# tuanggolt/hyperdrive

Hardware: AMD Instinct MI355X
Metric: verified consensus msgs/sec (secp256k1) at 1/2/4/8 MI355X; % INT32 VALU peak (higher is better)
Workload: dtype u32 (256-bit modular integer arithmetic)

## Files before the change

hyperdrive_amd/csrc/hd_fastverify.hip:

```cpp
#include <hip/hip_runtime.h>

#include <algorithm>
#include <cstdio>
#include <cstdlib>
#include <cstring>
#include <string>
#include <map>
#include <mutex>
#include <unordered_map>
#include <vector>

#include "../../include/hd_verify.h"
#include "hd_fixedbase.h"
#include "hd_dedup.h"
#include "hd_scmont.h"
#include "hd_internal.h"
#include "hd_verify_msg.h"

using namespace hd;

struct FbWork {
    const gp* gtab = nullptr;
    uint32_t nslots = 0;
    uint32_t max_slots = 0;
    gp** tabs = nullptr;
    std::vector<gp*> chunks;
    ge* base = nullptr;
    ge* pub = nullptr;
    uint32_t* state = nullptr;
    int32_t* adm_slot = nullptr;
    bool map_ok = true;
    size_t cap_adm_slot = 0;
    uint32_t* list = nullptr;
    uint32_t* counts = nullptr;
    uint32_t* zr = nullptr;
    struct Scratch {
        uint32_t* rows = nullptr;
        size_t cap_rows = 0;
        uint32_t* dtab = nullptr;
        size_t cap_dtab = 0;
        uint32_t* slow = nullptr;
        size_t cap_slow = 0;
        uint32_t* count = nullptr;
        uint32_t* slow2 = nullptr;
        size_t cap_slow2 = 0;
        hipEvent_t done = nullptr;
        hipStream_t stream = nullptr;
        bool used = false;
    };
    static constexpr int NSCRATCH = 3;
    Scratch sc[NSCRATCH];
    int next = 0;
    int last_set = -1;
    uint32_t* nr_host = nullptr;
    uint32_t* nr_dev = nullptr;
    uint32_t* est_host = nullptr;
    uint32_t* est_dev = nullptr;
    unsigned long long* dstats = nullptr;
    hipEvent_t done = nullptr;
    hipStream_t last = nullptr;
    bool any = false;
    bool steady = false;
    bool prof = false;
    std::vector<hipEvent_t> ev_call, ev_sums;
    size_t n_call = 0, n_sums = 0;
    std::unordered_map<std::string, uint32_t> slot_of;
    std::vector<uint32_t> free_slots;
    uint32_t used = 1;
    int wp = HD_FB_W;
    int last_k = 8;
    double budget = 0;
    size_t bytes = 0;
    uint32_t* fdict = nullptr;
    uint32_t* fnext = nullptr;
    uint32_t fbase = 0, fcap = 0, fres = 0;
    uint32_t* fpend_host = nullptr;
    uint32_t* fpend_dev = nullptr;
    uint32_t fseen = 0;
    uint32_t* fhit = nullptr;
    ge* fkey = nullptr;
    uint32_t fwait = 1, fcalls = 0;
    bool fforce = false;
    uint32_t evictions = 0;
    uint32_t evict_checks = 0;
    uint32_t evict_aborts = 0;
};

namespace {

#define FBCHK(expr, what)                                \
    do {                                                 \
        hipError_t e_ = (expr);                          \
        if (e_ != hipSuccess) return hd_ctx_fail(ctx, e_, what); \
    } while (0)

struct FastSrc {
    const DevBatch& b;
    uint32_t i;
    const uint8_t* dg;
    __device__ __forceinline__ uint32_t type() const { return b.type[i]; }
    __device__ __forceinline__ uint32_t value(int w) const { return load_be32(b.value32 + 32 * (size_t)i + 4 * w); }
    __device__ __forceinline__ uint32_t from(int w) const { return load_be32(b.from32 + 32 * (size_t)i + 4 * w); }
    __device__ __forceinline__ uint32_t sig_r(int w) const { return load_be32(b.sig65 + 65 * (size_t)i + 4 * w); }
    __device__ __forceinline__ uint32_t sig_s(int w) const { return load_be32(b.sig65 + 65 * (size_t)i + 32 + 4 * w); }
    __device__ __forceinline__ uint32_t sig_v() const { return b.sig65[65 * (size_t)i + 64]; }
    __device__ __forceinline__ void sig(uint32_t r_be[8], uint32_t s_be[8], uint32_t& v) const {
        load_sig65(r_be, s_be, v, b.sig65, i, b.n);
    }
    __device__ __forceinline__ void from_words(uint32_t w[8]) const { load_row32_be(w, b.from32, i); }
    __device__ __forceinline__ void value_words(uint32_t w[8]) const { load_row32_be(w, b.value32, i); }
};

#define HD_FAST_LIVE 0xFDu

template <int NW>
HD void soa_load(uint32_t (&w)[NW], const uint32_t* __restrict__ p, uint32_t n, uint32_t i) {
    HD_UNROLL for (int k = 0; k < NW; k++) w[k] = p[(size_t)k * n + i];
}
template <int NW>
HD void soa_store(uint32_t* __restrict__ p, uint32_t n, uint32_t i, const uint32_t (&w)[NW]) {
    HD_UNROLL for (int k = 0; k < NW; k++) p[(size_t)k * n + i] = w[k];
}

struct SplitRows {
    uint32_t* aux;
    int32_t* idx;
    uint32_t* ref;
    uint32_t* u1;
    uint32_t* u2;
    uint32_t* s;
    uint32_t* pre;
    uint32_t* xyz;
    uint32_t* cnt;
    int prio;
};

HD uint32_t dd_resolve(const SplitRows& rows, uint32_t i, uint32_t& c, bool& has_slot) {
    uint32_t rf = rows.ref[i];
    has_slot = (rf >> 30) != 3u;
    c = 0;
    if (!has_slot) return rf & 0xFFu;
    if (rf & HD_DD_REPEAT) rf = rows.ref[rf & HD_DD_INDEX];
    c = rf;
    return rows.aux[c] & 0xFFu;
}

HD void wave_prio(int p) {
    if (p == 1) __builtin_amdgcn_s_setprio(1);
    else if (p == 2) __builtin_amdgcn_s_setprio(2);
    else if (p >= 3) __builtin_amdgcn_s_setprio(3);
}

#define HD_REF_NEG 0x80000000u
#define HD_REF_ZERO 0x40000000u
#define HD_REF_IDX 0x3FFFFFFFu
template <int W>
HD uint32_t fb_ref(int d, int w) {
    const uint32_t ad = (uint32_t)(d < 0 ? -d : d);
    const uint32_t base = (uint32_t)w * FbL<W>::N;
    return d == 0 ? (base | HD_REF_ZERO) : ((base + ad - 1) | (d < 0 ? HD_REF_NEG : 0u));
}

__global__ __launch_bounds__(256) void k_fast_prep(DevBatch b, const uint8_t* __restrict__ digest_in,
                                                   const uint32_t* __restrict__ state,
                                                   const int32_t* __restrict__ adm_slot, AdmIndex ix,
                                                   uint32_t n_adm, SplitRows rows, const uint32_t* __restrict__ fdict,
                                                   uint32_t* __restrict__ fhit, uint32_t fbase,
                                                   uint32_t* __restrict__ dtab, uint32_t dmask) {
    wave_prio(rows.prio);
    const uint32_t i = blockIdx.x * blockDim.x + threadIdx.x;
    const uint32_t n = b.n;
    const bool present = i < n;
    FastSrc src{b, present ? i : 0u, digest_in};
    const uint32_t type = present ? src.type() : 0u;
    uint32_t code = HD_NEEDS_SLOW, slot = 0, rep = HD_DD_EMPTY;
    int32_t idx = -1;
    sc r, s, m;
    if (!present) {
    } else if (type < 1 || type > 3) {
        code = V_BAD_TYPE;
    } else {
        uint32_t from_be[8];
        src.from_words(from_be);
        idx = n_adm ? adm_index_find(ix, from_be) : -1;
        int32_t sl = idx >= 0 ? adm_slot[idx] : -1;
        if (idx < 0 && fdict) {
            sl = fdict_find(fdict, from_be);
            if (sl >= 0) idx = -2;
        }
        if (sl >= 0 && state[sl] == HD_FB_READY) {
            slot = (uint32_t)sl;
            if (idx == -2) atomicAdd(&fhit[sl - (int32_t)fbase], 1u);
            FastIn in;
            DdKey me;
            me.height = me.round = 0;
            if (digest_in) {
                load_row32_be(in.digest_be, digest_in, i);
                HD_UNROLL for (int k = 0; k < 8; k++) me.value[k] = in.digest_be[k];
            } else {
                src.value_words(me.value);
                me.height = b.height[i];
                me.round = b.round[i];
                if (type == T_PROPOSE)
                    sha256_propose(in.digest_be, me.height, me.round, b.valid_round ? b.valid_round[i] : -1, me.value);
                else
                    sha256_vote(in.digest_be, me.height, me.round, me.value);
            }
            src.sig(in.r_be, in.s_be, in.v);
            in.ready = true;
            fe x;
            uint8_t o;
            if (fast_prefix(o, r, s, m, x, in)) {
                code = HD_FAST_LIVE;
                if (dtab && type != T_PROPOSE) {
                    HD_UNROLL for (int k = 0; k < 8; k++) {
                        me.from[k] = from_be[k];
                        me.r[k] = in.r_be[k];
                        me.s[k] = in.s_be[k];
                    }
                    me.v = in.v;
                    const uint32_t h = dd_hash(me);
                    HD_NOUNROLL for (uint32_t p = 0; p < HD_DD_PROBES; p++) {
                        const uint32_t cur = atomicCAS(&dtab[(h + p) & dmask], HD_DD_EMPTY, i);
                        if (cur == HD_DD_EMPTY) break;
                        DdKey other;
                        dd_key_load(other, b.height, b.round, b.value32, digest_in, b.from32, b.sig65, cur, n);
                        if (dd_key_equal(me, other)) {
                            rep = cur;
                            break;
                        }
                    }
                }
            } else {
                code = o;
            }
        }
    }
    const bool live = code == HD_FAST_LIVE;
    const bool distinct = live && rep == HD_DD_EMPTY;
    __shared__ uint32_t s_cnt[4], s_base;
    const uint32_t lane = threadIdx.x & 63u, wv = threadIdx.x >> 6;
    const unsigned long long bd = __ballot(distinct), br = __ballot(live && !distinct);
    if (lane == 0) s_cnt[wv] = (uint32_t)__popcll(bd) | (uint32_t)__popcll(br) << 16;
    __syncthreads();
    if (threadIdx.x == 0) {
        const uint32_t t = s_cnt[0] + s_cnt[1] + s_cnt[2] + s_cnt[3];
        s_base = 0;
        if (t)
            s_base = (uint32_t)atomicAdd((unsigned long long*)(rows.cnt + 2),
                                         (unsigned long long)(t & 0xFFFFu) | (unsigned long long)(t >> 16) << 32);
    }
    __syncthreads();
    if (!present) return;
    if (distinct) {
        uint32_t c = s_base + (uint32_t)__popcll(bd & ((1ull << lane) - 1ull));
        for (uint32_t w = 0; w < wv; w++) c += s_cnt[w] & 0xFFFFu;
        rows.aux[c] = slot << 8 | HD_FAST_LIVE;
        soa_store(rows.u1, n, c, m.v);
        soa_store(rows.u2, n, c, r.v);
        soa_store(rows.s, n, c, s.v);
        rows.ref[i] = c;
    } else {
        rows.ref[i] = live ? (HD_DD_REPEAT | rep) : (HD_DD_FINAL | code);
    }
    rows.idx[i] = idx;
}

template <int K>
HD uint32_t split_lanes(uint32_t nc) {
    return ((nc + (uint32_t)K - 1) / (uint32_t)K + 63u) & ~63u;
}

template <int K>
__global__ __launch_bounds__(256) void k_fast_sinv(uint32_t n, SplitRows rows, uint32_t* __restrict__ est,
                                                   unsigned long long* __restrict__ stats) {
    wave_prio(rows.prio);
    const uint32_t t = blockIdx.x * blockDim.x + threadIdx.x;
    const uint32_t nc = rows.cnt[2], T = split_lanes<K>(nc);
    if (t == 0) {
        const uint32_t reps = rows.cnt[3];
        if (est) {
            est[1] = n;
            est[0] = nc;
        }
        if (nc + reps) atomicAdd(&stats[0], (unsigned long long)nc + reps);
        if (reps) atomicAdd(&stats[1], (unsigned long long)reps);
    }
    if (t >= T) return;
    sc sv[K];
    uint32_t live = 0;
    static_for<K>([&](auto jc) {
        constexpr int j = decltype(jc)::value;
        const uint32_t i = (uint32_t)j * T + t;
        const uint32_t ic = i < nc ? i : nc - 1;
        const uint32_t a = rows.aux[ic];
        soa_load(sv[j].v, rows.s, n, ic);
        live |= (i < nc && (a & 0xFFu) == HD_FAST_LIVE) ? 1u << j : 0u;
    });
    if (!live) return;
    sm pre[K], acc;
    HD_UNROLL for (int k = 0; k < 9; k++) acc.n[k] = 0;
    static_for<K>([&](auto jc) {
        constexpr int j = decltype(jc)::value;
        if ((live >> j) & 1u) {
            sm ss;
            sm_from_sc(ss, sv[j]);
            if (live & ((1u << j) - 1u)) sm_mul(acc, acc, ss);
            else acc = ss;
        }
        pre[j] = acc;
    });
    sm inv;
    {
        sc p, pinv;
        sm_to_sc(p, acc);
        sc_inv_divsteps(pinv, p);
        sm_from_sc(inv, pinv);
        sm r2;
        sm_r2(r2);
        sm_mul(inv, inv, r2);
    }
    static_for<K>([&](auto jc) {
        constexpr int j = K - 1 - decltype(jc)::value;
        if (!((live >> j) & 1u)) return;
        const uint32_t i = (uint32_t)j * T + t;
        if (j > 0 && (live & ((1u << j) - 1u))) {
            sm sinv, ss;
            sm_mul(sinv, inv, pre[j > 0 ? j - 1 : 0]);
            sm_from_sc(ss, sv[j]);
            sm_mul(inv, inv, ss);
            soa_store(rows.pre, n, i, sinv.n);
        } else {
            soa_store(rows.pre, n, i, inv.n);
        }
    });
}

template <bool FIRST>
HD void sum_add(gxz& dst, const gxz& src, bool& started, const ge& p0, const ge& g, uint32_t ec) {
    const bool nz = !(ec & HD_REF_ZERO);
    const bool rare = __ballot(!(started && nz)) != 0ull;
    gxz_sum_step<FIRST>(dst, src, started, p0, g, (ec & HD_REF_NEG) != 0, nz, rare);
}

template <int WP>
HD void fast_digit_refs(uint32_t* dst, size_t stride, const SplitRows& rows, uint32_t n, uint32_t i) {
    sm sinv, x;
    soa_load(sinv.n, rows.pre, n, i);
    sc u;
    soa_load(u.v, rows.u1, n, i);
    sm_from_sc(x, u);
    sm_mul(x, x, sinv);
    sm_to_sc(u, x);
    HD_UNROLL for (int w = 0; w < FbL<HD_FB_WG>::NWIN; w++)
        dst[(size_t)w * stride] = fb_ref<HD_FB_WG>(fb_digit<HD_FB_WG>(u, w), w);
    soa_load(u.v, rows.u2, n, i);
    sm_from_sc(x, u);
    sm_mul(x, x, sinv);
    sm_to_sc(u, x);
    HD_UNROLL for (int w = 0; w < FbL<WP>::NWIN; w++)
        dst[(size_t)(FbL<HD_FB_WG>::NWIN + w) * stride] = fb_ref<WP>(fb_digit<WP>(u, w), w);
}

#if defined(__HIP_DEVICE_COMPILE__)
typedef __attribute__((address_space(1))) const gp gp_global;
#else
typedef const gp gp_global;
#endif

template <int WAVES, int WP, int PF>
__global__ __launch_bounds__(256, WAVES) void k_fast_sums(uint32_t n, const gp* __restrict__ gtab,
                                                          const gp* const* __restrict__ tabs, SplitRows rows) {
    constexpr int NG = FbL<HD_FB_WG>::NWIN, NT = NG + FbL<WP>::NWIN;
    static_assert(PF >= 0 && PF <= 2, "prefetch depth");
    __shared__ uint32_t sdig[NT * 256];
    const uint32_t i = blockIdx.x * blockDim.x + threadIdx.x;
    if (i >= rows.cnt[2]) return;
    const uint32_t a = rows.aux[i];
    if ((a & 0xFFu) != HD_FAST_LIVE) return;
    const gp_global* gt = (const gp_global*)gtab;
    const gp_global* pt = (const gp_global*)tabs[a >> 8];
    const size_t dstride = 256;
    const uint32_t* dp = sdig + threadIdx.x;
    fast_digit_refs<WP>(sdig + threadIdx.x, 256, rows, n, i);
    uint32_t e = dp[0];
    gxz acc;
    ge p0;
    gp_unpack(p0, gt[e & HD_REF_IDX]);
    if (e & HD_REF_NEG) fe_neg(p0.y, p0.y);
    fe_norm_weak(p0.y);
    gxz_set_ge(acc, p0);
    bool started = !(e & HD_REF_ZERO);
    auto tab = [&](int w) { return w < NG ? gt : pt; };
    auto dig = [&](int w) { return dp[(size_t)(w < NT - 1 ? w : NT - 1) * dstride]; };
    uint32_t c1 = dig(1), c2 = 0, dn = 0;
    gp q1, q2;
    if (PF > 0) q1 = gt[c1 & HD_REF_IDX];
    if (PF == 2) {
        c2 = dig(2);
        q2 = tab(2)[c2 & HD_REF_IDX];
    }
    if (PF > 0) dn = dig(PF + 1);
    auto advance = [&](int j, gp& cur, uint32_t& ec) {
        if (PF == 0) {
            ec = j == 1 ? c1 : dig(j);
            cur = tab(j)[ec & HD_REF_IDX];
            return;
        }
        cur = q1;
        ec = c1;
        if (PF == 2) {
            q1 = q2;
            c1 = c2;
            c2 = dn;
            q2 = tab(j + 2 < NT ? j + 2 : NT - 1)[c2 & HD_REF_IDX];
        } else {
            c1 = dn;
            q1 = tab(j + 1 < NT ? j + 1 : NT - 1)[c1 & HD_REF_IDX];
        }
        dn = dig(j + PF + 1);
    };
    gxz b;
    auto step = [&](int j, gxz& dst, const gxz& src) {
        gp cur;
        uint32_t ec;
        advance(j, cur, ec);
        ge g;
        gp_unpack(g, cur);
        if (j == 1) sum_add<true>(dst, src, started, p0, g, ec);
        else sum_add<false>(dst, src, started, p0, g, ec);
    };
    step(1, b, acc);
    HD_NOUNROLL for (int j = 2; j + 1 < NT; j += 2) {
        step(j, acc, b);
        step(j + 1, b, acc);
    }
    if constexpr ((NT - 2) % 2 == 1) step(NT - 1, acc, b);
    else acc = b;
    if (!started || gxz_is_inf(acc)) {
        rows.aux[i] = (a & ~0xFFu) | HD_NEEDS_SLOW;
        return;
    }
    fe xn, yn, t;
    gxz_finish(xn, yn, t, acc);
    soa_store(rows.xyz, n, i, xn.n);
    soa_store(rows.xyz + 9 * (size_t)n, n, i, yn.n);
    soa_store(rows.xyz + 18 * (size_t)n, n, i, t.n);
}

template <int K>
__global__ __launch_bounds__(256) void k_fast_zinv(uint32_t n, SplitRows rows) {
    static_assert(K >= 2 && (K & (K - 1)) == 0, "K: a power of two");
    wave_prio(rows.prio);
    const uint32_t t = blockIdx.x * blockDim.x + threadIdx.x;
    const uint32_t nc = rows.cnt[2], T = split_lanes<K>(nc);
    if (t >= T) return;
    const uint32_t* zrow = rows.xyz + 18 * (size_t)n;
    fe node[2 * K];
    uint32_t live = 0;
    static_for<K>([&](auto jc) {
        constexpr int j = decltype(jc)::value;
        const uint32_t i = (uint32_t)j * T + t;
        const uint32_t ic = i < nc ? i : nc - 1;
        const uint32_t a = rows.aux[ic];
        fe z;
        soa_load(z.n, zrow, n, ic);
        const bool on = i < nc && (a & 0xFFu) == HD_FAST_LIVE;
        live |= on ? 1u << j : 0u;
        HD_UNROLL for (int k = 1; k < 9; k++) z.n[k] = on ? z.n[k] : 0u;
        z.n[0] = on ? z.n[0] : 1u;
        node[K + j] = z;
    });
    if (!live) return;
    static_for<K - 1>([&](auto ic) {
        constexpr int i = K - 1 - decltype(ic)::value;
        fe_mul(node[i], node[2 * i], node[2 * i + 1]);
    });
    fe_inv_divsteps(node[1], node[1]);
    static_for<K - 1>([&](auto ic) {
        constexpr int i = 1 + decltype(ic)::value;
        fe a, b;
        fe_mul(a, node[i], node[2 * i + 1]);
        fe_mul(b, node[i], node[2 * i]);
        node[2 * i] = a;
        node[2 * i + 1] = b;
    });
    static_for<K>([&](auto jc) {
        constexpr int j = decltype(jc)::value;
        if ((live >> j) & 1u) soa_store(rows.pre, n, (uint32_t)j * T + t, node[K + j].n);
    });
}

HD void fast_rx(fe& x, const sc& r, uint32_t v) {
    uint32_t xw[8];
    HD_UNROLL for (int k = 0; k < 8; k++) xw[k] = r.v[k];
    if (v & 2) {
        const uint32_t N[8] = {HD_N0, HD_N1, HD_N2, HD_N3, HD_N4, 0xFFFFFFFFu, 0xFFFFFFFFu, 0xFFFFFFFFu};
        uint64_t c = 0;
        HD_UNROLL for (int k = 0; k < 8; k++) { c += (uint64_t)xw[k] + N[k]; xw[k] = (uint32_t)c; c >>= 32; }
    }
    fe_from_le(x, xw);
}

__device__ __forceinline__ void cmp_one(const DevBatch& b, const SplitRows& rows, const int32_t* __restrict__ adm_perm,
                       uint8_t* __restrict__ verdict, uint8_t* __restrict__ rec32, int32_t* __restrict__ signer,
                       uint32_t* __restrict__ slow, uint32_t* __restrict__ n_slow, uint32_t* __restrict__ bitmap,
                       bool auth, uint32_t i, bool present, const fe* zi) {
    const uint32_t n = b.n;
    uint8_t v = HD_NEEDS_SLOW;
    if (present) {
        uint32_t c;
        bool has_slot;
        v = (uint8_t)dd_resolve(rows, i, c, has_slot);
        if (v == HD_FAST_LIVE) {
            fe xn, yn, w, x;
            soa_load(xn.n, rows.xyz, n, c);
            soa_load(yn.n, rows.xyz + 9 * (size_t)n, n, c);
            if (zi) w = *zi;
            else soa_load(w.n, rows.pre, n, c);
            sc r;
            soa_load(r.v, rows.u2, n, c);
            const uint32_t sv = b.sig65[65 * (size_t)i + 64];
            fast_rx(x, r, sv);
            v = fast_final_xz(xn, yn, w, x, sv);
            if (auth && v == HD_NEEDS_SLOW) v = V_NOT_AUTHENTIC;
            if (v == V_VALID && rows.idx[i] == -2) v = V_NOT_ADMITTED;
        }
        if (v != HD_NEEDS_SLOW) {
            const bool ok = v == V_VALID;
            verdict[i] = v;
            if (rec32) {
                uint32_t f[8] = {0, 0, 0, 0, 0, 0, 0, 0};
                if (ok || (v == V_NOT_ADMITTED && rows.idx[i] == -2)) load_row32_be(f, b.from32, i);
                store_row32_be(rec32, i, f);
            }
            if (signer) signer[i] = ok ? adm_perm[rows.idx[i]] : -1;
        }
    }
    const bool to_slow = present && v == HD_NEEDS_SLOW;
    const unsigned long long bal = __ballot(to_slow);
    const uint32_t lane = threadIdx.x & 63u;
    if (bal) {
        const uint32_t leader = (uint32_t)__ffsll((long long)bal) - 1;
        uint32_t base = 0;
        if (lane == leader) base = atomicAdd(n_slow, (uint32_t)__popcll(bal));
        base = __shfl(base, (int)leader);
        if (to_slow) slow[base + (uint32_t)__popcll(bal & ((1ull << lane) - 1))] = i;
    }
    if (bitmap) {
        const unsigned long long ok = __ballot(present && v == V_VALID);
        const uint32_t i0 = i - lane;
        if (lane == 0 && i0 < n) {
            bitmap[i0 >> 5] = (uint32_t)ok;
            if (i0 + 32 < n) bitmap[(i0 >> 5) + 1] = (uint32_t)(ok >> 32);
        }
    }
}

__global__ __launch_bounds__(256) void k_fast_cmp(DevBatch b, SplitRows rows, const int32_t* __restrict__ adm_perm,
                                                  uint8_t* __restrict__ verdict, uint8_t* __restrict__ rec32,
                                                  int32_t* __restrict__ signer, uint32_t* __restrict__ slow,
                                                  uint32_t* __restrict__ n_slow, uint32_t* __restrict__ bitmap,
                                                  bool auth) {
    wave_prio(rows.prio);
    const uint32_t i = blockIdx.x * blockDim.x + threadIdx.x;
    cmp_one(b, rows, adm_perm, verdict, rec32, signer, slow, n_slow, bitmap, auth, i, i < b.n, nullptr);
}

__global__ __launch_bounds__(256) void k_slow_lift(DevBatch b, const uint32_t* __restrict__ list,
                                                   const uint32_t* __restrict__ count, uint8_t* __restrict__ verdict,
                                                   uint8_t* __restrict__ rec32, int32_t* __restrict__ signer,
                                                   uint32_t* __restrict__ out, uint32_t* __restrict__ n_out,
                                                   int prio, uint32_t* __restrict__ est, SplitRows rows,
                                                   const gp* __restrict__ gtab) {
    wave_prio(prio);
    const uint32_t total = *count, stride = gridDim.x * blockDim.x;
    if (est && blockIdx.x == 0 && threadIdx.x == 0) est[0] = total;
    const uint32_t lane = threadIdx.x & 63u;
    for (uint32_t base = blockIdx.x * blockDim.x; base < total; base += stride) {
        const uint32_t p = base + threadIdx.x;
        bool keep = false;
        uint32_t i = 0;
        if (p < total) {
            i = list[p];
            uint32_t r_be[8], s_be[8], v;
            load_sig65(r_be, s_be, v, b.sig65, i, b.n);
            sc r, s;
            fe x;
            uint8_t pre = sig_prefix(r, s, x, r_be, s_be, v);
            if (pre == V_VALID) {
                fe y2, y, seven;
                fe_sqr(y2, x);
                fe_mul(y2, y2, x);
                fe_set_u32(seven, 7);
                fe_add(y2, y2, seven);
                if (!fe_sqrt(y, y2)) {
                    pre = V_NO_POINT;
                } else if (gtab && rows.aux) {
                    uint32_t c;
                    bool has_slot;
                    if (dd_resolve(rows, i, c, has_slot) == HD_FAST_LIVE) {
                        ge R;
                        R.x = x;
                        R.y = y;
                        if (fe_is_odd(y) != ((v & 1u) != 0)) fe_neg(R.y, y);
                        sc m;
                        soa_load(m.v, rows.u1, b.n, c);
                        if (fb_is_infinity<HD_FB_WG>(m, s, R, GpTab{gtab})) pre = V_INFINITY;
                    }
                }
            }
            keep = pre == V_VALID;
            if (!keep) {
                verdict[i] = pre;
                if (rec32) {
                    const uint32_t z[8] = {0, 0, 0, 0, 0, 0, 0, 0};
                    store_row32_be(rec32, i, z);
                }
                if (signer) signer[i] = -1;
            }
        }
        const unsigned long long bal = __ballot(keep);
        if (bal) {
            const uint32_t leader = (uint32_t)__ffsll((long long)bal) - 1;
            uint32_t o = 0;
            if (lane == leader) o = atomicAdd(n_out, (uint32_t)__popcll(bal));
            o = __shfl(o, (int)leader);
            if (keep) out[o + (uint32_t)__popcll(bal & ((1ull << lane) - 1ull))] = i;
        }
    }
}

__global__ void k_fb_list(uint32_t nslots, const uint32_t* __restrict__ state, uint32_t* __restrict__ list,
                          uint32_t* __restrict__ count) {
    __shared__ uint32_t c;
    if (threadIdx.x == 0) c = 0;
    __syncthreads();
    for (uint32_t k = threadIdx.x; k < nslots; k += blockDim.x)
        if (state[k] == HD_FB_LEARNED) list[atomicAdd(&c, 1u)] = k;
    __syncthreads();
    if (threadIdx.x == 0) *count = c;
}

template <int W>
__global__ __launch_bounds__(256) void k_fb_bases(const uint32_t* __restrict__ list, const uint32_t* __restrict__ count,
                                                  const ge* __restrict__ pub, ge* __restrict__ base) {
    constexpr int NW = FbL<W>::NWIN;
    const uint32_t total = *count * NW;
    for (uint32_t t = blockIdx.x * blockDim.x + threadIdx.x; t < total; t += gridDim.x * blockDim.x) {
        const uint32_t slot = list[t / NW], j = t % NW;
        ge o;
        fb_window_base(o, pub[slot], W, (int)j);
        base[(size_t)slot * NW + j] = o;
    }
}

#define HD_FB_RUN 32
#define HD_FB_SEG 512
#define HD_FB_CHUNK 8
template <int W>
__global__ __launch_bounds__(256) void k_fb_runs(const uint32_t* __restrict__ list, const uint32_t* __restrict__ count,
                                                 const ge* __restrict__ base, gp* const* __restrict__ tabs,
                                                 uint32_t* __restrict__ zr_scratch) {
    constexpr uint32_t N = FbL<W>::N, NW = FbL<W>::NWIN;
    constexpr uint32_t SW = N / HD_FB_SEG;
    constexpr uint32_t SB = (NW - 1) * SW + FbL<W>::NTOP / HD_FB_SEG;
    static_assert(N % HD_FB_SEG == 0 && FbL<W>::NTOP % HD_FB_SEG == 0 && HD_FB_SEG % HD_FB_RUN == 0, "segments");
    const uint32_t T = gridDim.x * blockDim.x;
    const uint32_t tid = blockIdx.x * blockDim.x + threadIdx.x;
    const uint64_t total = (uint64_t)*count * SB;
    for (uint64_t g = tid; g < total; g += T) {
        const uint32_t slot = list[g / SB];
        const uint32_t rem = (uint32_t)(g % SB);
        const uint32_t j = min(rem / SW, NW - 1);
        const uint32_t d0 = 1 + (rem - j * SW) * HD_FB_SEG;
        const ge B = base[(size_t)slot * NW + j];
        gp* out = tabs[slot] + (size_t)j * N + (d0 - 1);
        gej a;
        uint32_t k0 = 0;
        if (d0 == 1) {
            gp q;
            gp_pack(q, B);
            out[0] = q;
            gej b;
            gej_set_ge(b, B);
            gej_dbl(a, b);
            k0 = 1;
        } else {
            fb_mul_small(a, B, d0);
        }
        for (uint32_t blk = 0; blk < HD_FB_SEG; blk += HD_FB_RUN) {
            const uint32_t lo = blk + (blk == 0 ? k0 : 0), hi = blk + HD_FB_RUN;
            HD_NOUNROLL for (uint32_t k = lo; k < hi; k++) {
                if (k > lo) {
                    fe zr;
                    gej_add_ge_zr(a, a, B, zr);
                    HD_UNROLL for (int w = 0; w < 9; w++)
                        zr_scratch[((size_t)(k - 1 - blk) * 9 + w) * T + tid] = zr.n[w];
                }
                fe x = a.x, y = a.y;
                fe_normalize(x);
                fe_normalize(y);
                gp q;
                fe_to_le(q.x, x);
                fe_to_le(q.y, y);
                out[k] = q;
            }
            fe zinv;
            fe_inv_divsteps(zinv, a.z);
            HD_NOUNROLL for (uint32_t k = hi; k-- > lo;) {
                ge p;
                gp_unpack(p, out[k]);
                fe z2, ax, ay;
                fe_sqr(z2, zinv);
                fe_mul(ax, p.x, z2);
                fe_mul(z2, z2, zinv);
                fe_mul(ay, p.y, z2);
                fe_normalize(ax);
                fe_normalize(ay);
// ... 169 lines not shown
    f->fcalls = 0;
    int rq = hd_fb_quiesce(ctx);
    if (rq) return rq;
    *miss = 0;
    f->evict_checks++;
    hipStream_t s = ctx->stream;
    const uint32_t B = HD_FD_BUCKETS, R = f->fres;
    std::vector<uint32_t> fd(HD_FD_WORDS), hit(64 + B), st(R);
    std::vector<ge> key(B), pub(R);
    FBCHK(hipMemcpyAsync(fd.data(), f->fdict, 4 * (size_t)HD_FD_WORDS, hipMemcpyDeviceToHost, s), "evict read");
    FBCHK(hipMemcpyAsync(hit.data(), f->fhit, 4 * hit.size(), hipMemcpyDeviceToHost, s), "evict read");
    FBCHK(hipMemcpyAsync(key.data(), f->fkey, sizeof(ge) * B, hipMemcpyDeviceToHost, s), "evict read");
    FBCHK(hipMemcpyAsync(pub.data(), f->pub + f->fbase, sizeof(ge) * R, hipMemcpyDeviceToHost, s), "evict read");
    FBCHK(hipMemcpyAsync(st.data(), f->state + f->fbase, 4 * (size_t)R, hipMemcpyDeviceToHost, s), "evict read");
    FBCHK(hipStreamSynchronize(s), "evict read");
    struct Ent {
        uint32_t from[8];
        uint32_t slot, hits;
        ge key;
        bool moved;
    };
    std::vector<Ent> held, loose;
    for (uint32_t b = 0; b < B; b++) {
        if (fd[b] != 2u) continue;
        Ent e;
        memcpy(e.from, &fd[2 * B + 8 * b], 32);
        e.slot = fd[B + b];
        e.moved = false;
        if (e.slot != 0xFFFFFFFFu && e.slot >= f->fbase && e.slot < f->fbase + R) {
            e.hits = hit[e.slot - f->fbase];
            e.key = pub[e.slot - f->fbase];
            held.push_back(e);
        } else {
            e.slot = 0xFFFFFFFFu;
            e.hits = hit[64 + b];
            e.key = key[b];
            loose.push_back(e);
        }
    }
    std::stable_sort(loose.begin(), loose.end(), [](const Ent& a, const Ent& b) { return a.hits > b.hits; });
    std::vector<Ent*> cold;
    for (Ent& e : held)
        if (st[e.slot - f->fbase] == HD_FB_READY) cold.push_back(&e);
    std::stable_sort(cold.begin(), cold.end(), [](const Ent* a, const Ent* b) { return a->hits < b->hits; });
    std::vector<Ent> promoted;
    size_t swaps = 0;
    while (swaps < loose.size() && swaps < cold.size() && loose[swaps].hits >= 2 * cold[swaps]->hits + 4) {
        Ent& hot = loose[swaps];
        Ent* old = cold[swaps];
        hot.slot = old->slot;
        hot.moved = true;
        old->slot = 0xFFFFFFFFu;
        old->moved = true;
        promoted.push_back(hot);
        swaps++;
    }
    std::vector<Ent> keep;
    for (const Ent& e : held) keep.push_back(e);
    for (const Ent& e : loose)
        if (e.moved || e.hits > 0) keep.push_back(e);
    std::stable_partition(keep.begin(), keep.end(), [](const Ent& e) { return e.slot != 0xFFFFFFFFu; });
    const bool dropped = keep.size() < held.size() + loose.size();
    if (swaps == 0 && !dropped) {
        f->fwait = std::min(2 * f->fwait, HD_FD_EVICT_WAIT_MAX);
        FBCHK(hipMemsetAsync(f->fhit, 0, 4 * hit.size(), s), "evict counters");
        FBCHK(hipStreamSynchronize(s), "evict counters");
        return HD_OK;
    }
    std::vector<uint32_t> nd(HD_FD_WORDS, 0u), efrom(8 * keep.size() + 8), eslot(keep.size() + 1);
    std::vector<int32_t> where(keep.size() + 1);
    for (size_t k = 0; k < keep.size(); k++) {
        memcpy(&efrom[8 * k], keep[k].from, 32);
        eslot[k] = keep[k].slot;
    }
    if (!fdict_rebuild(nd.data(), where.data(), efrom.data(), eslot.data(), (uint32_t)keep.size())) {
        f->evict_aborts++;
        f->fwait = std::min(2 * f->fwait, HD_FD_EVICT_WAIT_MAX);
        FBCHK(hipMemsetAsync(f->fhit, 0, 4 * hit.size(), s), "evict counters");
        FBCHK(hipStreamSynchronize(s), "evict counters");
        return HD_OK;
    }
    std::vector<ge> nkey(B);
    for (size_t k = 0; k < keep.size(); k++)
        if (where[k] >= 0) nkey[where[k]] = keep[k].key;
    FBCHK(hipMemcpyAsync(f->fdict, nd.data(), 4 * (size_t)HD_FD_WORDS, hipMemcpyHostToDevice, s), "evict write");
    FBCHK(hipMemcpyAsync(f->fkey, nkey.data(), sizeof(ge) * B, hipMemcpyHostToDevice, s), "evict write");
    FBCHK(hipMemsetAsync(f->fhit, 0, 4 * hit.size(), s), "evict counters");
    const uint32_t learned = HD_FB_LEARNED;
    for (const Ent& e : promoted) {
        FBCHK(hipMemcpyAsync(f->pub + e.slot, &e.key, sizeof(ge), hipMemcpyHostToDevice, s), "evict key");
        FBCHK(hipMemcpyAsync(f->state + e.slot, &learned, 4, hipMemcpyHostToDevice, s), "evict state");
    }
    FBCHK(hipStreamSynchronize(s), "evict write");
    f->fwait = swaps ? 1u : std::min(2 * f->fwait, HD_FD_EVICT_WAIT_MAX);
    f->fforce = swaps > 0;
    f->evictions += (uint32_t)swaps;
    *changed = true;
    return HD_OK;
}

}

static std::mutex g_fb_g_mutex;
static std::map<int, gp*> g_fb_g_tables;

static int fb_g_table(hd_ctx* ctx, const gp** out) {
    std::lock_guard<std::mutex> lock(g_fb_g_mutex);
    auto it = g_fb_g_tables.find(ctx->device);
    if (it != g_fb_g_tables.end()) {
        *out = it->second;
        return HD_OK;
    }
    ge g;
    const uint32_t GX[8] = {0x79BE667Eu, 0xF9DCBBACu, 0x55A06295u, 0xCE870B07u,
                            0x029BFCDBu, 0x2DCE28D9u, 0x59F2815Bu, 0x16F81798u};
    const uint32_t GY[8] = {0x483ADA77u, 0x26A3C465u, 0x5DA4FBFCu, 0x0E1108A8u,
                            0xFD17B448u, 0xA6855419u, 0x9C47D08Fu, 0xFB10D4B8u};
    fe_from_be(g.x, GX);
    fe_from_be(g.y, GY);
    gp* tab = nullptr;
    gp** tp = nullptr;
    ge *base = nullptr, *pub = nullptr;
    uint32_t* cl = nullptr;
    FBCHK(hipMalloc(&tab, sizeof(gp) * (size_t)FbL<HD_FB_WG>::TAB), "G table");
    FBCHK(hipMalloc(&tp, sizeof(gp*)), "G table pointer");
    FBCHK(hipMalloc(&base, sizeof(ge) * FbL<HD_FB_WG>::NWIN), "G bases");
    FBCHK(hipMalloc(&pub, sizeof(ge)), "G point");
    FBCHK(hipMalloc(&cl, 8), "G list");
    const uint32_t hl[2] = {0u, 1u};
    hipStream_t s = ctx->stream;
    FBCHK(hipMemcpyAsync(pub, &g, sizeof(ge), hipMemcpyHostToDevice, s), "G point");
    FBCHK(hipMemcpyAsync(cl, hl, 8, hipMemcpyHostToDevice, s), "G list");
    FBCHK(hipMemcpyAsync(tp, &tab, sizeof(gp*), hipMemcpyHostToDevice, s), "G table pointer");
    k_fb_bases<HD_FB_WG><<<1, 64, 0, s>>>(cl, cl + 1, pub, base);
    k_fb_runs<HD_FB_WG><<<fb_run_blocks(ctx), 256, 0, s>>>(cl, cl + 1, base, tp, ctx->fb->zr);
    FBCHK(hipGetLastError(), "G table kernels");
    FBCHK(hipStreamSynchronize(s), "G table build");
    (void)hipFree(base);
    (void)hipFree(pub);
    (void)hipFree(cl);
    (void)hipFree(tp);
    g_fb_g_tables[ctx->device] = tab;
    *out = tab;
    return HD_OK;
}

int hd_fb_init(hd_ctx* ctx) {
    if (ctx->fb) return HD_OK;
    ctx->fb = new (std::nothrow) FbWork();
    if (!ctx->fb) return HD_ENOMEM;
    FbWork* f = ctx->fb;
    f->budget = 64.0 * (1ull << 30);
    if (const char* m = getenv("HD_FB_MAX_BYTES")) f->budget = atof(m);
    f->max_slots = (uint32_t)std::max(1.0, std::min(1e6, f->budget / fb_slot_bytes(f->wp)));
    FBCHK(hipMalloc(&f->counts, 8), "fb counts");
    FBCHK(hipMalloc(&f->zr, fb_run_scratch_bytes(ctx)), "fb builder scratch");
    FBCHK(hipHostMalloc((void**)&f->nr_host, 4, hipHostMallocMapped | hipHostMallocCoherent), "fb ready count");
    *f->nr_host = 0xFFFFFFFFu;
    FBCHK(hipHostGetDevicePointer((void**)&f->nr_dev, f->nr_host, 0), "fb ready count map");
    FBCHK(hipHostMalloc((void**)&f->est_host, 16, hipHostMallocMapped | hipHostMallocCoherent), "fb list estimate");
    f->est_host[0] = f->est_host[1] = f->est_host[2] = f->est_host[3] = 0xFFFFFFFFu;
    FBCHK(hipHostGetDevicePointer((void**)&f->est_dev, f->est_host, 0), "fb list estimate map");
    FBCHK(hipHostMalloc((void**)&f->fpend_host, 8, hipHostMallocMapped | hipHostMallocCoherent), "fb foreign claims");
    f->fpend_host[0] = f->fpend_host[1] = 0;
    FBCHK(hipHostGetDevicePointer((void**)&f->fpend_dev, f->fpend_host, 0), "fb foreign claims map");
    FBCHK(hipMalloc(&f->dstats, 16), "fb repeat counters");
    FBCHK(hipMemset(f->dstats, 0, 16), "fb repeat counters clear");
    int rc = fb_alloc_slots(ctx);
    if (rc) return rc;
    return fb_g_table(ctx, &f->gtab);
}

const gp* hd_fb_gtab(const hd_ctx* ctx) { return ctx && ctx->fb ? ctx->fb->gtab : nullptr; }

void hd_fb_release(hd_ctx* ctx) {
    if (!ctx || !ctx->fb) return;
    FbWork* f = ctx->fb;
    fb_free_tables(ctx);
    if (f->done) (void)hipEventDestroy(f->done);
    for (hipEvent_t e : f->ev_call) (void)hipEventDestroy(e);
    for (hipEvent_t e : f->ev_sums) (void)hipEventDestroy(e);
    for (auto& sc : f->sc) {
        if (sc.done) (void)hipEventDestroy(sc.done);
        void* sp[] = {sc.rows, sc.slow, sc.count, sc.slow2, sc.dtab};
        for (void* p : sp)
            if (p) (void)hipFree(p);
    }
    void* ptrs[] = {f->counts, f->adm_slot, f->zr, f->fdict, f->fnext, f->fhit, f->fkey, f->dstats};
    for (void* p : ptrs)
        if (p) (void)hipFree(p);
    if (f->nr_host) (void)hipHostFree(f->nr_host);
    if (f->est_host) (void)hipHostFree(f->est_host);
    if (f->fpend_host) (void)hipHostFree(f->fpend_host);
    delete f;
    ctx->fb = nullptr;
}

static int split_k_for(const hd_ctx* ctx, uint32_t n) {
    const int k = ctx->var[HD_VAR_SPLIT_K];
    if (k > 0) return k;
    uint64_t lanes = n;
    if (const volatile uint32_t* est = ctx->fb->est_host) {
        const uint32_t seen = est[2], of = est[3];
        if (seen != 0xFFFFFFFFu && of != 0xFFFFFFFFu && seen != 0 && seen <= of) lanes = (uint64_t)n * seen / of;
    }
    return lanes >= (1u << 19) ? 16 : 8;
}

static double fb_free_cap(hd_ctx* ctx) {
    size_t fr = 0, tot = 0;
    (void)hipSetDevice(ctx->device);
    if (hipMemGetInfo(&fr, &tot) != hipSuccess) return 1e300;
    return 0.9 * (double)fr + (double)ctx->fb->bytes;
}

static int fb_pick_width(hd_ctx* ctx, uint32_t m, int cap) {
    if (ctx->var[HD_VAR_KEY_WIDTH]) return ctx->var[HD_VAR_KEY_WIDTH];
    FbWork* f = ctx->fb;
    const double others = (double)(fb_device_bytes(ctx->device) - std::min(fb_device_bytes(ctx->device), f->bytes));
    const double free_cap = fb_free_cap(ctx);
    const double shared = std::min(f->budget - others, free_cap);
    const double slots = (double)m + 1 + (ctx->var[HD_VAR_FOREIGN_KEYS] > 0 ? ctx->var[HD_VAR_FOREIGN_KEYS] : 0);
    const auto allowed = [cap](int w) { return cap == 0 || w <= cap; };
    if (allowed(HD_FB_WX) && fb_slot_bytes(HD_FB_WX) * slots <= shared) return HD_FB_WX;
    if (allowed(HD_FB_WW) && fb_slot_bytes(HD_FB_WW) * ((double)m + 1) <= shared) return HD_FB_WW;
    if (allowed(HD_FB_W) && fb_slot_bytes(HD_FB_W) * slots <= std::min(f->budget, free_cap)) return HD_FB_W;
    return HD_FB_WN;
}

static int fb_count_not_ready(hd_ctx* ctx) {
    FbWork* f = ctx->fb;
    uint32_t nr = 0;
    if (!f->slot_of.empty()) {
        std::vector<uint32_t> st(f->nslots);
        FBCHK(hipMemcpyAsync(st.data(), f->state, 4 * (size_t)f->nslots, hipMemcpyDeviceToHost, ctx->stream),
              "fb state read");
        FBCHK(hipStreamSynchronize(ctx->stream), "fb state read");
        for (const auto& kv : f->slot_of) nr += st[kv.second] != HD_FB_READY ? 1u : 0u;
    }
    *(volatile uint32_t*)f->nr_host = nr;
    return HD_OK;
}

static int fb_map(hd_ctx* ctx, const uint8_t* sorted, uint32_t m, int cap);

static bool fb_trace() {
    static const bool on = getenv("HD_FB_TRACE") != nullptr;
    return on;
}

static std::mutex g_fb_map_mutex[64];

int hd_fb_map_signatories(hd_ctx* ctx, const uint8_t* sorted, uint32_t m) {
    std::lock_guard<std::mutex> lock(g_fb_map_mutex[(unsigned)ctx->device % 64u]);
    int rc = HD_OK;
    for (int cap : {0, HD_FB_WW, HD_FB_W, HD_FB_WN}) {
        if (fb_trace()) {
            size_t fr = 0, tot = 0;
            (void)hipMemGetInfo(&fr, &tot);
            fprintf(stderr, "[fb] ctx %p m %u cap %d: wp %d nslots %u used %u max %u bytes %.2fG dev %.2fG free %.2fG\n",
                    (void*)ctx, m, cap, ctx->fb->wp, ctx->fb->nslots, ctx->fb->used, ctx->fb->max_slots,
                    ctx->fb->bytes / 1e9, fb_device_bytes(ctx->device) / 1e9, fr / 1e9);
        }
        rc = fb_map(ctx, sorted, m, cap);
        if (fb_trace())
            fprintf(stderr, "[fb] ctx %p -> rc %d wp %d nslots %u used %u %s\n", (void*)ctx, rc, ctx->fb->wp,
                    ctx->fb->nslots, ctx->fb->used, rc ? ctx->last_error.c_str() : "");
        if (rc != HD_ENOMEM || ctx->var[HD_VAR_KEY_WIDTH]) break;
        (void)hipGetLastError();
    }
    ctx->fb->map_ok = rc == HD_OK;
    return rc;
}

static int fb_map(hd_ctx* ctx, const uint8_t* sorted, uint32_t m, int cap) {
    FbWork* f = ctx->fb;
    int rq = hd_ctx_quiesce(ctx);
    if (rq) return rq;
    *(volatile uint32_t*)f->nr_host = 0xFFFFFFFFu;
    const int wp = fb_pick_width(ctx, m, cap);
    if (wp != f->wp || (cap && f->nslots < f->used)) {
        fb_free_tables(ctx);
        f->slot_of.clear();
        f->free_slots.clear();
        f->used = 1;
        f->fcap = f->fres = 0;
        f->wp = wp;
        f->max_slots =
            (uint32_t)std::max(1.0, std::min(1e6, std::min(f->budget, fb_free_cap(ctx)) / fb_slot_bytes(wp)));
        int ra = fb_alloc_slots(ctx);
        if (ra) return ra;
    }
    std::unordered_map<std::string, uint32_t> keep;
    std::vector<int32_t> adm_slot(std::max(m, 1u), -1);
    std::vector<uint32_t> fresh;
    for (uint32_t k = 0; k < m; k++) {
        std::string key(reinterpret_cast<const char*>(sorted + 32 * (size_t)k), 32);
        auto it = f->slot_of.find(key);
        if (it != f->slot_of.end()) {
            adm_slot[k] = (int32_t)it->second;
            keep.emplace(key, it->second);
            f->slot_of.erase(it);
        }
    }
    for (auto& kv : f->slot_of) {
        f->free_slots.push_back(kv.second);
        fresh.push_back(kv.second);
    }
    f->slot_of.swap(keep);
    for (uint32_t k = 0; k < m; k++) {
        if (adm_slot[k] >= 0) continue;
        uint32_t slot;
        if (!f->free_slots.empty()) {
            slot = f->free_slots.back();
            f->free_slots.pop_back();
        } else if (f->used < f->max_slots) {
            slot = f->used++;
        } else {
            continue;
        }
        adm_slot[k] = (int32_t)slot;
        f->slot_of.emplace(std::string(reinterpret_cast<const char*>(sorted + 32 * (size_t)k), 32), slot);
        fresh.push_back(slot);
    }
    const uint32_t want = (uint32_t)std::max(0, ctx->var[HD_VAR_FOREIGN_KEYS]);
    if (want && !f->fres && f->used + want <= f->max_slots) {
        f->fbase = f->used;
        f->fres = want;
        f->used += want;
    }
    f->fcap = std::min(want, f->fres);
    int rc = fb_grow_slots(ctx, f->used);
    if (rc) return rc;
    hipStream_t s = ctx->stream;
    for (uint32_t slot : fresh) FBCHK(hipMemsetAsync(f->state + slot, 0, 4, s), "fb slot reset");
    if (f->fres) {
        if (!f->fdict) FBCHK(hipMalloc(&f->fdict, 4 * (size_t)HD_FD_WORDS), "fb foreign dictionary");
        if (!f->fnext) FBCHK(hipMalloc(&f->fnext, 4), "fb foreign count");
        if (!f->fhit) FBCHK(hipMalloc(&f->fhit, 4 * (64 + (size_t)HD_FD_BUCKETS)), "fb foreign hits");
        if (!f->fkey) FBCHK(hipMalloc(&f->fkey, sizeof(ge) * HD_FD_BUCKETS), "fb foreign keys");
        FBCHK(hipMemsetAsync(f->fdict, 0, 4 * (size_t)HD_FD_WORDS, s), "fb foreign reset");
        FBCHK(hipMemsetAsync(f->fnext, 0, 4, s), "fb foreign reset");
        FBCHK(hipMemsetAsync(f->fhit, 0, 4 * (64 + (size_t)HD_FD_BUCKETS), s), "fb foreign reset");
        FBCHK(hipMemsetAsync(f->state + f->fbase, 0, 4 * (size_t)f->fres, s), "fb foreign reset");
        fb_foreign_forget(f);
    }
    rc = hd_dev_grow(ctx, (void**)&f->adm_slot, &f->cap_adm_slot, 4 * adm_slot.size());
    if (rc) return rc;
    FBCHK(hipMemcpyAsync(f->adm_slot, adm_slot.data(), 4 * adm_slot.size(), hipMemcpyHostToDevice, s), "fb adm_slot");
    FBCHK(hipStreamSynchronize(s), "fb map");
    return fb_count_not_ready(ctx);
}

int hd_fb_clear_keys(hd_ctx* ctx) {
    FbWork* f = ctx->fb;
    int rq = hd_ctx_quiesce(ctx);
    if (rq) return rq;
    if (f->nslots > 1) FBCHK(hipMemsetAsync(f->state + 1, 0, 4 * (size_t)(f->nslots - 1), ctx->stream), "fb clear");
    if (f->fres && f->fdict) {
        FBCHK(hipMemsetAsync(f->fdict, 0, 4 * (size_t)HD_FD_WORDS, ctx->stream), "fb clear");
        FBCHK(hipMemsetAsync(f->fnext, 0, 4, ctx->stream), "fb clear");
        FBCHK(hipMemsetAsync(f->fhit, 0, 4 * (64 + (size_t)HD_FD_BUCKETS), ctx->stream), "fb clear");
    }
    FBCHK(hipStreamSynchronize(ctx->stream), "fb clear");
    if (f->fres) fb_foreign_forget(f);
    return fb_count_not_ready(ctx);
}

static hipEvent_t* fb_prof_pair(std::vector<hipEvent_t>& ev, size_t& used, bool on) {
    if (!on) return nullptr;
    if (2 * (used + 1) > ev.size()) {
        hipEvent_t a = nullptr, b = nullptr;
        if (hipEventCreate(&a) != hipSuccess) return nullptr;
        if (hipEventCreate(&b) != hipSuccess) {
            (void)hipEventDestroy(a);
            return nullptr;
        }
        ev.push_back(a);
        ev.push_back(b);
    }
    return &ev[2 * used++];
}

static uint32_t fallback_blocks(uint32_t est, uint32_t full) {
    if (est == 0xFFFFFFFFu) return full;
    const uint64_t want = ((uint64_t)est * 5 / 4 + 255) / 256;
    return (uint32_t)std::min<uint64_t>(full, std::max<uint64_t>(want, std::min(64u, full)));
}

template <int WP>
static void launch_sums(const hd_ctx* ctx, uint32_t blocks, hipStream_t s, uint32_t n, const gp* gtab,
                        const gp* const* tab, const SplitRows& rows) {
    int w = ctx->var[HD_VAR_SUM_WAVES];
    const int pf = ctx->var[HD_VAR_SUM_PREFETCH];
    if (w == 0) w = (uint64_t)n < 2ull * 3 * 4 * 64 * (uint64_t)std::max(ctx->n_cu, 1) ? 4 : 3;
    if (pf == 2) {
        if (w == 2) k_fast_sums<2, WP, 2><<<blocks, 256, 0, s>>>(n, gtab, tab, rows);
        else k_fast_sums<3, WP, 2><<<blocks, 256, 0, s>>>(n, gtab, tab, rows);
    } else {
        if (w == 2) k_fast_sums<2, WP, 1><<<blocks, 256, 0, s>>>(n, gtab, tab, rows);
        else if (w == 4) k_fast_sums<4, WP, 0><<<blocks, 256, 0, s>>>(n, gtab, tab, rows);
        else k_fast_sums<3, WP, 1><<<blocks, 256, 0, s>>>(n, gtab, tab, rows);
    }
}

template <int K, int WP>
static void launch_split(hd_ctx* ctx, const DevBatch& b, const uint8_t* d_digest, uint8_t* d_verdict,
                         uint8_t* d_rec32, int32_t* d_signer, uint32_t* d_bitmap, const SplitRows& rows,
                         const FbWork::Scratch& sc, hipStream_t s, bool auth) {
    FbWork* f = ctx->fb;
    const uint32_t n = b.n;
    const uint32_t tb = (split_lanes<K>(n) + 255) / 256, nb = (n + 255) / 256;
    uint32_t* dtab = ctx->var[HD_VAR_DEDUP] ? sc.dtab : nullptr;
    k_fast_prep<<<nb, 256, 0, s>>>(b, d_digest, f->state, f->adm_slot, hd_adm_index(ctx), ctx->n_adm, rows,
                                   f->fcap ? f->fdict : nullptr, f->fhit, f->fbase, dtab, dd_table_words(n) - 1u);
    k_fast_sinv<K><<<tb, 256, 0, s>>>(n, rows, f->est_dev + 2, f->dstats);
    hipEvent_t* pe = fb_prof_pair(f->ev_sums, f->n_sums, f->prof);
    if (pe) (void)hipEventRecord(pe[0], s);
    launch_sums<WP>(ctx, nb, s, n, f->gtab, f->tabs, rows);
    if (pe) (void)hipEventRecord(pe[1], s);
    k_fast_zinv<K><<<tb, 256, 0, s>>>(n, rows);
    k_fast_cmp<<<nb, 256, 0, s>>>(b, rows, ctx->d_adm_perm, d_verdict, d_rec32, d_signer, sc.slow, sc.count,
                                  d_bitmap, auth);
}

static int fb_verify_impl(hd_ctx* ctx, const DevBatch& b, const uint8_t* d_digest, uint8_t* d_verdict,
                          uint8_t* d_rec32, int32_t* d_signer, uint32_t* d_bitmap, FbWork::Scratch& sc,
                          hipStream_t s, bool auth);

int hd_fb_verify(hd_ctx* ctx, const DevBatch& b, const uint8_t* d_digest, uint8_t* d_verdict, uint8_t* d_rec32,
                 int32_t* d_signer, uint32_t* d_bitmap, hipStream_t s, bool auth) {
    FbWork* f = ctx->fb;
    if (!f->done) FBCHK(hipEventCreateWithFlags(&f->done, hipEventDisableTiming), "fb event");
    const int j = f->next;
    f->next = (j + 1) % FbWork::NSCRATCH;
    FbWork::Scratch& sc = f->sc[j];
    if (!sc.done) FBCHK(hipEventCreateWithFlags(&sc.done, hipEventDisableTiming), "fb scratch event");
    if (!sc.count) FBCHK(hipMalloc(&sc.count, 16), "fb scratch count");
    bool evicted = false;
    int re = fb_evict(ctx, &evicted);
    if (re) return re;
    const bool steady = !evicted && f->nr_host && *(volatile uint32_t*)f->nr_host == 0 && !fb_foreign_pending(f);
// ... 226 lines not shown
```

Measured before the change: 1.015 billion.

## Fuse final x/z check into z-inverse kernel and store verdict bytes

The batched z-inverse kernel now runs the final affine-x comparison itself, prefetching x, y and r for the next element, and writes a one-word verdict per distinct row instead of a 9-limb inverse. The recovery bits v are packed into the top of the aux word so they no longer have to be reread from the signature. The compare kernel then only reads ref and pre words rather than x, y, inverse and r rows. This cuts global traffic and lets the compare kernel follow repeats cheaply, but it caps the slot index below the packed v bits and adds register pressure in the zinv kernel.

```diff
diff --git a/hyperdrive_amd/csrc/hd_fastverify.hip b/hyperdrive_amd/csrc/hd_fastverify.hip
--- a/hyperdrive_amd/csrc/hd_fastverify.hip
+++ b/hyperdrive_amd/csrc/hd_fastverify.hip
@@ -112,6 +112,11 @@
 };
 
 #define HD_FAST_LIVE 0xFDu
+#define HD_AUX_V_SHIFT 30
+#define HD_AUX_SLOT_MASK ((1u << (HD_AUX_V_SHIFT - 8)) - 1u)
+#define HD_FB_SLOT_LIMIT 1000000u
+static_assert(HD_FB_SLOT_LIMIT <= HD_AUX_SLOT_MASK, "a table slot fits below the recovery bits of aux");
+
 
 template <int NW>
 HD void soa_load(uint32_t (&w)[NW], const uint32_t* __restrict__ p, uint32_t n, uint32_t i) {
@@ -174,6 +179,7 @@
     FastSrc src{b, present ? i : 0u, digest_in};
     const uint32_t type = present ? src.type() : 0u;
     uint32_t code = HD_NEEDS_SLOW, slot = 0, rep = HD_DD_EMPTY;
+    uint32_t me_v = 0;
     int32_t idx = -1;
     sc r, s, m;
     if (!present) {
@@ -208,6 +214,7 @@
             }
             src.sig(in.r_be, in.s_be, in.v);
             in.ready = true;
+            me_v = in.v;
             fe x;
             uint8_t o;
             if (fast_prefix(o, r, s, m, x, in)) {
@@ -255,7 +262,7 @@
     if (distinct) {
         uint32_t c = s_base + (uint32_t)__popcll(bd & ((1ull << lane) - 1ull));
         for (uint32_t w = 0; w < wv; w++) c += s_cnt[w] & 0xFFFFu;
-        rows.aux[c] = slot << 8 | HD_FAST_LIVE;
+        rows.aux[c] = me_v << HD_AUX_V_SHIFT | slot << 8 | HD_FAST_LIVE;
         soa_store(rows.u1, n, c, m.v);
         soa_store(rows.u2, n, c, r.v);
         soa_store(rows.s, n, c, s.v);
@@ -379,7 +386,7 @@
     const uint32_t a = rows.aux[i];
     if ((a & 0xFFu) != HD_FAST_LIVE) return;
     const gp_global* gt = (const gp_global*)gtab;
-    const gp_global* pt = (const gp_global*)tabs[a >> 8];
+    const gp_global* pt = (const gp_global*)tabs[(a >> 8) & HD_AUX_SLOT_MASK];
     const size_t dstride = 256;
     const uint32_t* dp = sdig + threadIdx.x;
     fast_digit_refs<WP>(sdig + threadIdx.x, 256, rows, n, i);
@@ -448,6 +455,17 @@
     soa_store(rows.xyz + 18 * (size_t)n, n, i, t.n);
 }
 
+HD void fast_rx(fe& x, const sc& r, uint32_t v) {
+    uint32_t xw[8];
+    HD_UNROLL for (int k = 0; k < 8; k++) xw[k] = r.v[k];
+    if (v & 2) {
+        const uint32_t N[8] = {HD_N0, HD_N1, HD_N2, HD_N3, HD_N4, 0xFFFFFFFFu, 0xFFFFFFFFu, 0xFFFFFFFFu};
+        uint64_t c = 0;
+        HD_UNROLL for (int k = 0; k < 8; k++) { c += (uint64_t)xw[k] + N[k]; xw[k] = (uint32_t)c; c >>= 32; }
+    }
+    fe_from_le(x, xw);
+}
+
 template <int K>
 __global__ __launch_bounds__(256) void k_fast_zinv(uint32_t n, SplitRows rows) {
     static_assert(K >= 2 && (K & (K - 1)) == 0, "K: a power of two");
@@ -458,6 +476,7 @@
     const uint32_t* zrow = rows.xyz + 18 * (size_t)n;
     fe node[2 * K];
     uint32_t live = 0;
+    uint64_t vbits = 0;
     static_for<K>([&](auto jc) {
         constexpr int j = decltype(jc)::value;
         const uint32_t i = (uint32_t)j * T + t;
@@ -467,11 +486,18 @@
         soa_load(z.n, zrow, n, ic);
         const bool on = i < nc && (a & 0xFFu) == HD_FAST_LIVE;
         live |= on ? 1u << j : 0u;
+        vbits |= (uint64_t)(a >> HD_AUX_V_SHIFT) << (2 * j);
         HD_UNROLL for (int k = 1; k < 9; k++) z.n[k] = on ? z.n[k] : 0u;
         z.n[0] = on ? z.n[0] : 1u;
         node[K + j] = z;
     });
-    if (!live) return;
+    if (!live) {
+        static_for<K>([&](auto jc) {
+            const uint32_t i = (uint32_t)decltype(jc)::value * T + t;
+            if (i < nc) rows.pre[i] = HD_FAST_LIVE;
+        });
+        return;
+    }
     static_for<K - 1>([&](auto ic) {
         constexpr int i = K - 1 - decltype(ic)::value;
         fe_mul(node[i], node[2 * i], node[2 * i + 1]);
@@ -485,45 +511,46 @@
         node[2 * i] = a;
         node[2 * i + 1] = b;
     });
+    fe xn[2], yn[2];
+    sc r[2];
+    auto fetch = [&](int j, int q) {
+        const uint32_t i = (uint32_t)j * T + t;
+        const uint32_t ic = i < nc ? i : nc - 1;
+        soa_load(xn[q].n, rows.xyz, n, ic);
+        soa_load(yn[q].n, rows.xyz + 9 * (size_t)n, n, ic);
+        soa_load(r[q].v, rows.u2, n, ic);
+    };
+    fetch(0, 0);
     static_for<K>([&](auto jc) {
-        constexpr int j = decltype(jc)::value;
-        if ((live >> j) & 1u) soa_store(rows.pre, n, (uint32_t)j * T + t, node[K + j].n);
+        constexpr int j = decltype(jc)::value, q = j & 1;
+        if (j + 1 < K) fetch(j + 1, q ^ 1);
+        const uint32_t i = (uint32_t)j * T + t;
+        uint32_t res = HD_FAST_LIVE;
+        if ((live >> j) & 1u) {
+            const uint32_t v = (vbits >> (2 * j)) & 3u;
+            fe x;
+            fast_rx(x, r[q], v);
+            res = fast_final_xz(xn[q], yn[q], node[K + j], x, v);
+        }
+        if (i < nc) rows.pre[i] = res;
     });
-}
-
-HD void fast_rx(fe& x, const sc& r, uint32_t v) {
-    uint32_t xw[8];
-    HD_UNROLL for (int k = 0; k < 8; k++) xw[k] = r.v[k];
-    if (v & 2) {
-        const uint32_t N[8] = {HD_N0, HD_N1, HD_N2, HD_N3, HD_N4, 0xFFFFFFFFu, 0xFFFFFFFFu, 0xFFFFFFFFu};
-        uint64_t c = 0;
-        HD_UNROLL for (int k = 0; k < 8; k++) { c += (uint64_t)xw[k] + N[k]; xw[k] = (uint32_t)c; c >>= 32; }
-    }
-    fe_from_le(x, xw);
 }
 
 __device__ __forceinline__ void cmp_one(const DevBatch& b, const SplitRows& rows, const int32_t* __restrict__ adm_perm,
                        uint8_t* __restrict__ verdict, uint8_t* __restrict__ rec32, int32_t* __restrict__ signer,
                        uint32_t* __restrict__ slow, uint32_t* __restrict__ n_slow, uint32_t* __restrict__ bitmap,
-                       bool auth, uint32_t i, bool present, const fe* zi) {
+                       bool auth, uint32_t i, bool present) {
     const uint32_t n = b.n;
     uint8_t v = HD_NEEDS_SLOW;
     if (present) {
-        uint32_t c;
-        bool has_slot;
-        v = (uint8_t)dd_resolve(rows, i, c, has_slot);
-        if (v == HD_FAST_LIVE) {
-            fe xn, yn, w, x;
-            soa_load(xn.n, rows.xyz, n, c);
-            soa_load(yn.n, rows.xyz + 9 * (size_t)n, n, c);
-            if (zi) w = *zi;
-            else soa_load(w.n, rows.pre, n, c);
-            sc r;
-            soa_load(r.v, rows.u2, n, c);
-            const uint32_t sv = b.sig65[65 * (size_t)i + 64];
-            fast_rx(x, r, sv);
-            v = fast_final_xz(xn, yn, w, x, sv);
+        uint32_t rf = rows.ref[i];
+        if ((rf >> 30) == 3u) {
+            v = (uint8_t)(rf & 0xFFu);
+        } else {
+            if (rf & HD_DD_REPEAT) rf = rows.ref[rf & HD_DD_INDEX];
+            v = (uint8_t)rows.pre[rf];
             if (auth && v == HD_NEEDS_SLOW) v = V_NOT_AUTHENTIC;
+            if (v == HD_FAST_LIVE) v = HD_NEEDS_SLOW;
             if (v == V_VALID && rows.idx[i] == -2) v = V_NOT_ADMITTED;
         }
         if (v != HD_NEEDS_SLOW) {
@@ -564,7 +591,7 @@
                                                   bool auth) {
     wave_prio(rows.prio);
     const uint32_t i = blockIdx.x * blockDim.x + threadIdx.x;
-    cmp_one(b, rows, adm_perm, verdict, rec32, signer, slow, n_slow, bitmap, auth, i, i < b.n, nullptr);
+    cmp_one(b, rows, adm_perm, verdict, rec32, signer, slow, n_slow, bitmap, auth, i, i < b.n);
 }
 
 __global__ __launch_bounds__(256) void k_slow_lift(DevBatch b, const uint32_t* __restrict__ list,
@@ -1040,7 +1067,7 @@
     FbWork* f = ctx->fb;
     f->budget = 64.0 * (1ull << 30);
     if (const char* m = getenv("HD_FB_MAX_BYTES")) f->budget = atof(m);
-    f->max_slots = (uint32_t)std::max(1.0, std::min(1e6, f->budget / fb_slot_bytes(f->wp)));
+    f->max_slots = (uint32_t)std::max(1.0, std::min((double)HD_FB_SLOT_LIMIT, f->budget / fb_slot_bytes(f->wp)));
     FBCHK(hipMalloc(&f->counts, 8), "fb counts");
     FBCHK(hipMalloc(&f->zr, fb_run_scratch_bytes(ctx)), "fb builder scratch");
     FBCHK(hipHostMalloc((void**)&f->nr_host, 4, hipHostMallocMapped | hipHostMallocCoherent), "fb ready count");
@@ -1175,7 +1202,7 @@
         f->fcap = f->fres = 0;
         f->wp = wp;
         f->max_slots =
-            (uint32_t)std::max(1.0, std::min(1e6, std::min(f->budget, fb_free_cap(ctx)) / fb_slot_bytes(wp)));
+            (uint32_t)std::max(1.0, std::min((double)HD_FB_SLOT_LIMIT, std::min(f->budget, fb_free_cap(ctx)) / fb_slot_bytes(wp)));
         int ra = fb_alloc_slots(ctx);
         if (ra) return ra;
     }
```

After: 1.019 billion (median of 2 runs). About the same (+0.4%).
